# mankeyboy/ASR-FeatExt-OpenCL

Hardware: NVIDIA B200
Metric: mfcc_delta_delta2_frames_per_s (higher is better)
Workload: dtype f32

## Files before the change

asr-featext-opencl_b200/csrc/afe_batch.cu:

```cuda
#include <algorithm>
#include <atomic>
#include <memory>
#include <cmath>
#include <cstdlib>
#include <cstring>

#include "afe_internal.h"
#include "afe_fused_host.h"
#include "afe_nccl.h"

namespace afe {

void FftTables::build(int n2)
{
    release();
    N2 = n2;
    const int M = n2 / 2, R = M / 16;
    std::vector<float2> a((size_t)R * 16), p((size_t)M / 2);
    for (int l = 0; l < R; l++)
        for (int k1 = 0; k1 < 16; k1++) {
            const double ang = -2.0 * M_PI * (double)(l * k1) / (double)M;
            a[(size_t)l * 16 + k1] = make_float2((float)cos(ang), (float)sin(ang));
        }
    for (int k = 0; k < M / 2; k++) {
// ... 97 lines not shown

__global__ void k_normalize_tiles(float *__restrict__ out, const Tile *__restrict__ tiles, int width, int norm_type,
                                  const float *__restrict__ mean, const float *__restrict__ scale)
{
    extern __shared__ float s_ms[];
    dev::normalise_tile_rows(out, tiles[blockIdx.x], width, norm_type, mean, scale, s_ms);
}

static std::atomic<int> g_launches{0};
int kernel_launch_count() { return g_launches.load(); }
void count_launch(int n) { g_launches.fetch_add(n); }

#define AFE_DECL_INST(k) cudaError_t fused_launch_##k(const FusedLaunch &); int fused_max_clusters_##k(const FusedLaunch &);
#define AFE_FOR_EACH_INST(X) X(0) X(1) X(2) X(3) X(4) X(5) X(6) X(7) X(8) X(9) X(10) X(11) X(12) X(13) X(14) X(15) X(16) X(17) \
    X(18) X(19) X(20) X(21) X(22) X(23)
AFE_FOR_EACH_INST(AFE_DECL_INST)
#undef AFE_DECL_INST

cudaError_t launch_fused_variant(int key, const FusedLaunch &fl)
{
    typedef cudaError_t (*fn_t)(const FusedLaunch &);
#define AFE_ENTRY(k) fused_launch_##k,
    static const fn_t table[kFusedVariants] = {AFE_FOR_EACH_INST(AFE_ENTRY)};
#undef AFE_ENTRY
    if (key < 0 || key >= kFusedVariants) return cudaErrorInvalidValue;
    return table[key](fl);
}
int fused_variant_max_clusters(int key, const FusedLaunch &fl)
{
    typedef int (*fn_t)(const FusedLaunch &);
#define AFE_ENTRY(k) fused_max_clusters_##k,
    static const fn_t table[kFusedVariants] = {AFE_FOR_EACH_INST(AFE_ENTRY)};
#undef AFE_ENTRY
    if (key < 0 || key >= kFusedVariants) return -1;
    return table[key](fl);
}

std::string fused_unsupported_reason(const Derived &d)
{
    if (d.N2 != 512 && d.N2 != 256) return "fused path supports 256/512-point FFTs (window_size 129..512)";
    if (d.S % 2) return "fused path needs an even shift";
    if (d.dct_len > 16) return "fused path supports ceps_len + c0 <= 16";
    if (d.width > 128) return "fused path supports output width <= 128";
    if (d.nb > kMaxBanks) return "fused path supports num_banks <= 64";
    if (d.W > 26 * (d.M / 16) && d.W > d.N2) return "window longer than the FFT";
    return "";
}

static void build_mel_const(const Derived &d, float alpha, MelConst &mc)
{
    std::vector<int> edges; std::vector<float> filters, dct;
    build_filters(d, alpha, edges, filters);
    for (int i = 0; i + 1 < (int)edges.size(); i++)
        if (edges[i + 1] < edges[i]) throw Error("mel filter edges are not monotonic");
    if (edges.front() < 0 || edges.back() > d.M) throw Error("mel filterbank exceeds the Nyquist bin (check low_freq/high_freq)");
    memset(&mc, 0, sizeof mc);
    int off4 = 0;
    const float scale = 0.5f / (float)d.N2;
    for (int w = 0; w < 8; w++) {
        mc.wstart[w] = (short)off4;
        for (int b = w; b < d.nb; b += 8) {
            const int j0 = edges[b], j1 = edges[b + 2], s4 = j0 & ~3, n8 = std::max(1, (j1 - s4 + 7) / 8);
            if (off4 + 2 * n8 > kMaxWl4) throw Error("mel weight list exceeds the kernel-parameter budget");
            if (s4 + 8 * n8 > kMagStride + 16) throw Error("mel filter too wide for the fused kernel");
            mc.desc[b] = (s4 / 4) | (n8 << 16);
            float *wt = reinterpret_cast<float *>(mc.wl4 + off4);
            for (int j = j0; j < j1; j++) wt[j - s4] = filters[(size_t)(b % 2) * d.N2 + j] * scale;
            off4 += 2 * n8;
        }
    }
    if (d.C > 0) {
        build_dct(d, dct);
        for (int k = 0; k < d.nb; k++)
            for (int j = 0; j < d.dct_len; j++) reinterpret_cast<float *>(mc.dct4[k])[j] = dct[(size_t)k * d.dct_len + j];
    }
}

FusedEngine::FusedEngine(const Derived &dd, int dev) : d(dd), device(dev)
{
    const std::string why = fused_unsupported_reason(d);
    if (!why.empty()) throw Error(why);
    sm_count = sm_count_of(dev);
    fft.build(d.N2);
    int tc = 512;
    tc = std::min(tc, (6912 / d.cols) / kRoundFrames * kRoundFrames);
    tc = std::max(tc, kRoundFrames * ((2 * d.D + 1 + kRoundFrames - 1) / kRoundFrames + 1));
    tc_max = tc; nout_max = tc - 2 * d.D;
    const int ns = d.width / d.cols;
    L = d.N2 == 512 ? fused_smem_layout<512>(8, d.S, d.cols, tc_max, nout_max, d.l2, ns)
                    : fused_smem_layout<256>(8, d.S, d.cols, tc_max, nout_max, d.l2, ns);
    if (L.total > 227 * 1024) throw Error("fused kernel shared-memory budget exceeded");
    const int R = d.M / 16;
    pruned = d.W <= 26 * R;
    const int kf = (d.nb + 7) / 8;
    key = (d.N2 == 512 ? 0 : 6) + (pruned ? 0 : 3) + (kf <= 3 ? 0 : kf <= 5 ? 1 : 2);
}
FusedEngine::~FusedEngine() { fft.release(); mel.release(); }

void FusedEngine::set_window(const float *window, cudaStream_t st)
{
    upload_window(d, window, mel, st);
    window_set = true;
}
void FusedEngine::ensure_mel(float alpha)
{
    if (mc_alpha != alpha) { build_mel_const(d, alpha, mc); mc_alpha = alpha; }
}
std::string FusedEngine::kernel_label() const
{
    const int kf = (d.nb + 7) / 8;
    char buf[96];
    snprintf(buf, sizeof buf, "k_fused_mfcc<%d,%d,8,%d,%s>", d.N2, pruned ? 13 : 16, kf <= 3 ? 3 : kf <= 5 ? 5 : 8,
             pre != 0.f ? "true" : "false");
    return buf;
}

int FusedEngine::latency_tile(int n_out) const
{
    const int target = std::max(1, 2 * sm_count);
    const int want = (n_out + target - 1) / target;
    const int rounds = std::max(2, (want + 2 * d.D + kRoundFrames - 1) / kRoundFrames);
    return std::max(1, std::min(nout_max, rounds * kRoundFrames - 2 * d.D));
}

void FusedEngine::plan_uniform(int T, int t_first, int n_out, int nout_cap, int &ntile, int &nout) const
{
    const int cap = nout_cap > 0 ? std::min(nout_cap, nout_max) : nout_max;
    int best_cost = 1 << 30;
    ntile = (n_out + cap - 1) / cap;
    for (int cand = ntile; cand <= ntile + 3; cand++) {
        const int no = (n_out + cand - 1) / cand;
        int cost = 0;
        for (int t0 = t_first; t0 < t_first + n_out; t0 += no) {
            const int c0 = std::max(0, t0 - d.D), c1 = std::min(T, t0 + std::min(no, t_first + n_out - t0) + d.D);
            cost += (c1 - c0 + kRoundFrames - 1) / kRoundFrames;
        }
        if (cost < best_cost) { best_cost = cost; ntile = cand; }
    }
    nout = (n_out + ntile - 1) / ntile;
    ntile = (n_out + nout - 1) / nout;
}

int FusedEngine::plan_rows(std::vector<Tile> &tiles, long long pcm_off, long long out_row0, int T, int t_first, int n_out,
                           int group, int nout_cap) const
{
    if (n_out <= 0) return 0;
    int count, nout;
    plan_uniform(T, t_first, n_out, nout_cap, count, nout);
    const int first = (int)tiles.size();
    for (int t0 = t_first; t0 < t_first + n_out; t0 += nout) {
        Tile tl;
        tl.pcm_off = pcm_off; tl.out_row0 = out_row0; tl.T = T; tl.t0 = t0;
        tl.nout = std::min(nout, t_first + n_out - t0); tl.group = group;
        tl.tile0 = first; tl.ntiles = count; tl.flags = 0; tl.pad_ = 0;
        tiles.push_back(tl);
    }
    return count;
}

FusedArgs FusedEngine::base_args(int q1, bool use_tma) const
{
    FusedArgs a{};
    a.window2 = mel.d_window2; a.tw_a = fft.d_tw_a; a.tw_p = fft.d_tw_p;
    a.norm_type = d.p.norm; a.norm_after_dyn = d.p.norm_after_dyn;
    a.W = d.W; a.S = d.S; a.nb = d.nb; a.dct_len = d.C > 0 ? d.dct_len : 0; a.cols = d.cols; a.width = d.width;
    a.l1 = d.l1; a.l2 = d.l2; a.nstreams = d.width / d.cols;
    a.q1 = d.D > 0 ? q1 : 0;
    a.use_tma = use_tma ? 1 : 0;
    a.tc_max = tc_max;
    a.pre = pre;
    float den1 = 0, den2 = 0;
    for (int l = 1; l <= d.l1; l++) den1 += l * l;
    for (int l = 1; l <= d.l2; l++) den2 += l * l;
    a.rden1 = den1 > 0 ? 1.f / (2 * den1) : 0.f;
// ... 516 lines not shown
```

asr-featext-opencl_b200/csrc/afe_fused.cuh:

```cuda
#pragma once
#include <cfloat>

#include "afe_fft.cuh"
#include "afe_internal.h"
#include "afe_mel.cuh"

namespace afe {

struct Tile {
    long long pcm_off;
    long long out_row0;
    int T;
    int t0;
    int nout;
    int group;
    int tile0;
    int ntiles;
    int flags;
    int pad_;
};
constexpr int kTileNoStats = 1;
constexpr int kTileQ1All = 2;

constexpr int kMaxBanks = 64;
constexpr int kMaxWl4 = (2 * 257 + 10 * kMaxBanks + 3) / 4;
constexpr int kMagStride = 260;
__host__ __device__ constexpr int mag_row(int f) { return 8 * (f >> 3) + ((f >> 1) & 3) + 4 * (f & 1); }

struct MelConst {
    float4 wl4[kMaxWl4];
    float4 dct4[kMaxBanks][4];
    int desc[kMaxBanks];
    short wstart[8];
};

struct FusedArgs {
    const int16_t *pcm;
    float *out;
    const Tile *tiles;
    const float2 *window2, *tw_a, *tw_p;
    double *partials;
    int *counters;
    int cluster_norm;
    int tile_base;
    int norm_type, norm_after_dyn;
#ifdef AFE_DEVTOOLS
    int debug_skip;
#endif
    int W, S, nb, dct_len, cols, width, l1, l2, nstreams;
    int q1;
    int use_tma;
    int stats_rows_mode;
    int stats_count;
    int use_last;
    float *g_mean, *g_scale;
    int *work_counter;
    unsigned *flags;
    unsigned epoch;
    int ntiles_launch;
    float pre;
    int blk_ntiles, blk_T, blk_t_first, blk_n_out, blk_nout, blk_spec, blk_spec_q1;
    int stats_kind;
    int tc_max;
    float rden1, rden2;
};

constexpr int kRoundFrames = 32;
constexpr int kMaxFusedThreads = 256;

struct FusedSmem {
    int off_mbar, off_mags, off_part, off_warp, warp_bytes, w_pcm, w_scratch, pcm_bytes, off_dhat, off_dd, off_red,
        off_cep, total;
};

inline int align_up(int v, int a) { return (v + a - 1) / a * a; }

template <int N2>
FusedSmem fused_smem_layout(int kFusedWarps, int S, int cols, int tc_max, int nout_max, int l2, int nstreams)
{
    using C = dev::FftCfg<N2>;
    const int kWarpFrames = kRoundFrames / kFusedWarps;
    FusedSmem L;
    int o = 0;
    L.off_mbar = o; o += align_up(kFusedWarps * 8, 16);
    L.off_mags = o; o += align_up((kRoundFrames * kMagStride + 16) * 4, 16);
    L.pcm_bytes = align_up(((kWarpFrames - 1) * S + N2) * 2, 16) + 16;
    L.w_pcm = 0;
    L.warp_bytes = L.pcm_bytes;
    o = align_up(o, 128);
    L.off_warp = o; o += kFusedWarps * L.warp_bytes;
    o = align_up(o, 128);
    const int scratch = kFusedWarps * align_up(C::FPW * C::SCR * 8, 16);
    const int part = kFusedWarps * 4 * kRoundFrames * 16;
    L.w_scratch = align_up(C::FPW * C::SCR * 8, 16);
    L.off_part = o; o += scratch > part ? scratch : part;
    const int dhat = nstreams >= 2 ? align_up((nout_max + 2 * l2) * cols * 4, 16) : 0;
    const int dd = nstreams >= 3 ? align_up(nout_max * cols * 4, 16) : 0;
    L.off_dhat = L.off_mags;
    L.off_dd = L.off_dhat + dhat;
    L.off_red = L.off_dd + dd;
    const int phase3_end = L.off_red + kMaxFusedThreads * 4 * 8;
    if (phase3_end > o) o = align_up(phase3_end, 128);
    L.off_cep = o; o += align_up(tc_max * cols * 4, 16);
    L.total = o;
    return L;
}

namespace dev {

__device__ __forceinline__ uint32_t smem_u32(const void *p) { return (uint32_t)__cvta_generic_to_shared(p); }

__device__ __forceinline__ void mbar_init(uint64_t *bar, int count)
{
    asm volatile("mbarrier.init.shared::cta.b64 [%0], %1;" ::"r"(smem_u32(bar)), "r"(count));
}
__device__ __forceinline__ void mbar_expect_tx(uint64_t *bar, uint32_t bytes)
{
    asm volatile("mbarrier.arrive.expect_tx.shared::cta.b64 _, [%0], %1;" ::"r"(smem_u32(bar)), "r"(bytes) : "memory");
}
__device__ __forceinline__ void mbar_wait(uint64_t *bar, uint32_t parity)
{
    for (uint32_t spin = 0; spin < (1u << 24); spin++) {
        uint32_t done;
        asm volatile(
            "{\n\t.reg .pred p;\n\t"
            "mbarrier.try_wait.parity.shared::cta.b64 p, [%1], %2;\n\t"
            "selp.u32 %0, 1, 0, p;\n\t}"
            : "=r"(done)
            : "r"(smem_u32(bar)), "r"(parity)
            : "memory");
        if (done) return;
    }
    __trap();
}
__device__ __forceinline__ void tma_bulk_g2s(void *dst, const void *src, uint32_t bytes, uint64_t *bar)
{
    asm volatile("cp.async.bulk.shared::cluster.global.mbarrier::complete_tx::bytes [%0], [%1], %2, [%3];" ::"r"(
                     smem_u32(dst)),
                 "l"(src), "r"(bytes), "r"(smem_u32(bar))
                 : "memory");
}

__device__ __forceinline__ float4 lds128(uint32_t addr)
{
    float4 v;
    asm volatile("ld.shared.v4.f32 {%0, %1, %2, %3}, [%4];" : "=f"(v.x), "=f"(v.y), "=f"(v.z), "=f"(v.w) : "r"(addr));
    return v;
}
__device__ __forceinline__ uint32_t opaque(uint32_t v)
{
    asm volatile("" : "+r"(v));
    return v;
}

__device__ __forceinline__ void cluster_sync()
{
    asm volatile("barrier.cluster.arrive.release.aligned;\n\tbarrier.cluster.wait.acquire.aligned;" ::: "memory");
}
__device__ __forceinline__ uint32_t cluster_size()
{
    uint32_t n;
    asm volatile("mov.u32 %0, %%cluster_nctarank;" : "=r"(n));
    return n;
}
__device__ __forceinline__ double ld_peer_f64(const double *local, uint32_t rank)
{
    uint32_t peer;
    double v;
    asm volatile("mapa.shared::cluster.u32 %0, %1, %2;" : "=r"(peer) : "r"(smem_u32(local)), "r"(rank));
    asm volatile("ld.shared::cluster.f64 %0, [%1];" : "=d"(v) : "r"(peer) : "memory");
    return v;
}

__device__ __forceinline__ int clampi(int v, int lo, int hi) { return v < lo ? lo : (v > hi ? hi : v); }

template <class Dst>
__device__ __forceinline__ void sum_row_groups(const double *rec, int rp, int width, int c, Dst dst)
{
    double s0 = 0.0, s1 = 0.0, lo = (double)FLT_MAX, hi = -(double)FLT_MAX;
    for (int g = 0; g < rp; g++) {
        const double *p = rec + (g * width + c) * 4;
        s0 += p[0]; s1 += p[1];
        lo = fmin(lo, p[2]); hi = fmax(hi, p[3]);
    }
    double *d = dst();
    d[0] = s0; d[1] = s1; d[2] = lo; d[3] = hi;
}

}

namespace dev {

__device__ __forceinline__ float delta_num(const float *p, int stride, int L)
{
    if (L == 3) {
        float num = p[stride] - p[-stride];
        num = fmaf(2.f, p[2 * stride] - p[-2 * stride], num);
        return fmaf(3.f, p[3 * stride] - p[-3 * stride], num);
    }
    float num = 0.f;
    for (int l = 1; l <= L; l++) num = fmaf((float)l, p[l * stride] - p[-l * stride], num);
    return num;
}

template <int KIND>
__device__ __forceinline__ void write_rows(float *__restrict__ orow, const float *__restrict__ src, int r_off, int rpp, int nout,
                                           int rq, int rs, int cols, int width, int D, double &sum, double &sumsq, float &mn,
                                           float &mx)
{
    const int ostep = rpp * width, sstep = rpp * cols;
    orow += r_off * width;
    src += r_off * cols;
    for (int r = r_off; r < nout; r += rpp, orow += ostep, src += sstep) {
        const float sval = *src;
        *orow = r >= rq ? src[-D * cols] : sval;
        if (KIND >= 1 && r < rs) {
            sum += (double)sval;
            if (KIND >= 2) sumsq += (double)__fmul_rn(sval, sval);
            if (KIND >= 3) { mn = fminf(mn, sval); mx = fmaxf(mx, sval); }
        }
    }
}

template <int MODE>
__device__ __forceinline__ void phase3_l3(const int KIND, const FusedArgs &a, const Tile &tl, const float *__restrict__ s_cep,
                                          int c0f, int c1f, double *__restrict__ s_red3, int tid, int nthreads, int rs,
                                          const float *norm3 = nullptr)
{
    constexpr int R = 8;
    const int cols = a.cols, width = a.width, T = tl.T, t0 = tl.t0, nout = tl.nout;
    const int rp = nthreads / cols, g = tid / cols, c = tid - g * cols;
    if (g >= rp) return;
    const int q1 = (tl.flags & kTileQ1All) ? 2 : a.q1;
    const int rq = q1 ? (q1 == 2 ? 0 : max(0, T - 6 - t0)) : nout;
    const float rden1 = a.rden1, rden2 = a.rden2;
    double sum[3] = {0.0, 0.0, 0.0}, sumsq[3] = {0.0, 0.0, 0.0};
    float mn[3] = {FLT_MAX, FLT_MAX, FLT_MAX}, mx[3] = {-FLT_MAX, -FLT_MAX, -FLT_MAX};
    float nm[3] = {0.f, 0.f, 0.f}, ns[3] = {1.f, 1.f, 1.f};
    if (MODE == 2) {
#pragma unroll
        for (int k = 0; k < 3; k++) { nm[k] = norm3[k]; ns[k] = norm3[3 + k]; }
    }
    const bool cmn = a.norm_type == AFE_NORM_CMN;
    float *obase = a.out + (tl.out_row0 + t0) * (long long)width + c;
    for (int r0 = g * R; r0 < (MODE == 1 ? rs : nout); r0 += rp * R) {
        float x[R + 12], dh[R + 6];
#pragma unroll
        for (int i = 0; i < R + 12; i++)
            x[i] = s_cep[(clampi(t0 + r0 - 6 + i, c0f, c1f - 1) - c0f) * cols + c];
#pragma unroll
        for (int j = 0; j < R + 6; j++) {
            float num = x[j + 4] - x[j + 2];
            num = fmaf(2.f, x[j + 5] - x[j + 1], num);
            num = fmaf(3.f, x[j + 6] - x[j], num);
            dh[j] = __fmul_rn(num, rden1);
        }
        float *orow = obase + (long long)r0 * width;
#pragma unroll
        for (int r = 0; r < R; r++, orow += width) {
            const int row = r0 + r;
            if (row >= nout) break;
            float num = dh[r + 4] - dh[r + 2];
            num = fmaf(2.f, dh[r + 5] - dh[r + 1], num);
            num = fmaf(3.f, dh[r + 6] - dh[r], num);
            const float v[3] = {x[r + 6], dh[r + 3], __fmul_rn(num, rden2)};
            if (MODE == 0) {
                orow[0] = row >= rq ? x[r] : v[0];
                orow[cols] = v[1];
                orow[2 * cols] = v[2];
            } else if (MODE == 2) {
                const float w0 = row >= rq ? x[r] : v[0];
                orow[0] = cmn ? w0 - nm[0] : (w0 - nm[0]) * ns[0];
                orow[cols] = cmn ? v[1] - nm[1] : (v[1] - nm[1]) * ns[1];
                orow[2 * cols] = cmn ? v[2] - nm[2] : (v[2] - nm[2]) * ns[2];
            }
            if (MODE != 2 && KIND >= 1 && row < rs) {
#pragma unroll
                for (int k = 0; k < 3; k++) {
                    sum[k] += (double)v[k];
                    if (KIND >= 2) sumsq[k] += (double)__fmul_rn(v[k], v[k]);
                    if (KIND >= 3) { mn[k] = fminf(mn[k], v[k]); mx[k] = fmaxf(mx[k], v[k]); }
                }
            }
        }
    }
    if (MODE != 2) {
#pragma unroll
        for (int k = 0; k < 3; k++) {
            double *p = s_red3 + ((g * width) + k * cols + c) * 4;
            p[0] = sum[k]; p[1] = sumsq[k]; p[2] = (double)mn[k]; p[3] = (double)mx[k];
        }
    }
}

}

namespace dev {
__device__ __forceinline__ Tile load_tile(const FusedArgs &a, int idx)
{
    if (a.blk_ntiles == 0) return a.tiles[idx];
    const int D = a.l1 + a.l2;
    Tile tl;
    tl.pcm_off = 0; tl.out_row0 = -(long long)a.blk_t_first; tl.T = a.blk_T; tl.group = 0; tl.tile0 = 0;
    tl.ntiles = a.blk_ntiles + a.blk_spec; tl.pad_ = 0;
    if (idx < a.blk_ntiles) {
        tl.t0 = a.blk_t_first + idx * a.blk_nout;
        tl.nout = min(a.blk_nout, a.blk_t_first + a.blk_n_out - tl.t0);
        tl.flags = 0;
    } else {
        tl.t0 = a.blk_T - D; tl.nout = D;
        tl.flags = kTileNoStats | (a.blk_spec_q1 ? kTileQ1All : 0);
    }
    return tl;
}

constexpr int kSeqTiles = 32, kSegs = 6;
__host__ __device__ inline int seg_len(int ntiles) { return ntiles <= kSeqTiles ? ntiles : (ntiles + kSegs - 1) / kSegs; }

static __device__ unsigned g_opaque_zero = 0;

__device__ __forceinline__ void sum_records(const double *__restrict__ partials, int width, int c, int t_begin, int t_end,
                                            double &s0, double &s1, double &lo, double &hi, int tstep = 1)
{
    s0 = 0.0; s1 = 0.0; lo = (double)FLT_MAX; hi = -(double)FLT_MAX;
    constexpr int U = 8;
    const size_t stride = (size_t)width * 4 * tstep;
    const double *p = partials + ((size_t)t_begin * width + c) * 4;
    const int last = t_end - 1;
    const unsigned z = *reinterpret_cast<volatile unsigned *>(&g_opaque_zero);
    for (int t = t_begin; t < t_end; t += U * tstep, p += U * stride) {
        double2 a[U], b[U];
#pragma unroll
        for (int k = 0; k < U; k++) {
            const double2 *q = reinterpret_cast<const double2 *>(t + k * tstep <= last ? p + k * stride : p);
            a[k] = q[0];
            b[k] = q[1];
        }
        unsigned all = 0;
#pragma unroll
        for (int k = 0; k < U; k++)
            all |= (unsigned)__double2hiint(a[k].x) | (unsigned)__double2hiint(a[k].y) | (unsigned)__double2hiint(b[k].x) |
                   (unsigned)__double2hiint(b[k].y);
        a[0].x = __hiloint2double(__double2hiint(a[0].x) | (int)(all & z), __double2loint(a[0].x));
#pragma unroll
        for (int k = 0; k < U; k++) {
            const bool ok = t + k * tstep <= last;
            s0 += ok ? a[k].x : 0.0; s1 += ok ? a[k].y : 0.0;
            lo = fmin(lo, ok ? b[k].x : (double)FLT_MAX); hi = fmax(hi, ok ? b[k].y : -(double)FLT_MAX);
        }
    }
}

__device__ __forceinline__ void group_total(const double *__restrict__ partials, int width, int tile0, int ntiles, int tid,
                                            int nthreads, double *s_seg, int c_of_tid, double &s0, double &s1, double &lo, double &hi)
{
    if (ntiles <= kSeqTiles) {
        if (tid < width) sum_records(partials, width, c_of_tid, tile0, tile0 + ntiles, s0, s1, lo, hi);
        return;
    }
    const int len = seg_len(ntiles);
    for (int i = tid; i < kSegs * width; i += nthreads) {
        const int seg = i / width, c = i - seg * width;
        const int b = min(ntiles, seg * len), e = min(ntiles, b + len);
        double a0, a1, l, h;
        sum_records(partials, width, c, tile0 + b, tile0 + e, a0, a1, l, h);
        double *o = s_seg + (size_t)i * 4;
        o[0] = a0; o[1] = a1; o[2] = l; o[3] = h;
    }
    __syncthreads();
    if (tid < width) {
        s0 = 0.0; s1 = 0.0; lo = (double)FLT_MAX; hi = -(double)FLT_MAX;
        for (int seg = 0; seg < kSegs; seg++) {
            const double *o = s_seg + ((size_t)seg * width + c_of_tid) * 4;
            s0 += o[0]; s1 += o[1];
            lo = fmin(lo, o[2]); hi = fmax(hi, o[3]);
        }
    }
}

__device__ __forceinline__ void normalise_tile_rows(float *__restrict__ out, const Tile &tl, int width, int norm_type,
                                                    const float *__restrict__ mean, const float *__restrict__ scale, float *s_ms)
{
    float *base = out + (tl.out_row0 + tl.t0) * (long long)width;
    const int n = tl.nout * width;
    for (int i = threadIdx.x; i < width; i += blockDim.x) {
        s_ms[i] = __ldcg(mean + (long long)tl.group * width + i);
        s_ms[width + i] = norm_type == AFE_NORM_CMN ? 1.f : __ldcg(scale + (long long)tl.group * width + i);
    }
    __syncthreads();
    const float *m = s_ms, *sc = s_ms + width;
    const bool cmn = norm_type == AFE_NORM_CMN;
    const int head = min(n, (int)(((16 - (reinterpret_cast<uintptr_t>(base) & 15)) & 15) >> 2));
    const int n4 = (n - head) >> 2, tail0 = head + 4 * n4;
    if ((int)threadIdx.x < head) {
        const int i = threadIdx.x;
        const float v = __ldcg(base + i) - m[i % width];
        base[i] = cmn ? v : v * sc[i % width];
    }
    if ((int)threadIdx.x < n - tail0) {
        const int i = tail0 + threadIdx.x, c = i % width;
        const float v = __ldcg(base + i) - m[c];
        base[i] = cmn ? v : v * sc[c];
    }
    float4 *p4 = reinterpret_cast<float4 *>(base + head);
    int c = (head + 4 * (int)threadIdx.x) % width;
    const int cstep = (4 * (int)blockDim.x) % width;
    constexpr int U = 4;
    const int bd = blockDim.x;
    for (int j = threadIdx.x; j < n4; j += U * bd) {
        float4 v[U];
#pragma unroll
        for (int k = 0; k < U; k++)
            if (j + k * bd < n4) v[k] = __ldcg(p4 + j + k * bd);
#pragma unroll
        for (int k = 0; k < U; k++) {
            if (j + k * bd < n4) {
                int c1 = c + 1; if (c1 >= width) c1 -= width;
                int c2 = c1 + 1; if (c2 >= width) c2 -= width;
                int c3 = c2 + 1; if (c3 >= width) c3 -= width;
                float4 w = v[k];
                w.x -= m[c]; w.y -= m[c1]; w.z -= m[c2]; w.w -= m[c3];
                if (!cmn) { w.x *= sc[c]; w.y *= sc[c1]; w.z *= sc[c2]; w.w *= sc[c3]; }
                p4[j + k * bd] = w;
            }
            c += cstep; if (c >= width) c -= width;
        }
    }
}

__device__ __forceinline__ void normalise_role(const FusedArgs &a, const Tile tl, float *s_ms)
{
    if (threadIdx.x == 0) {
        unsigned v = 0;
        for (unsigned spin = 0; spin < (1u << 26); spin++) {
            asm volatile("ld.acquire.gpu.global.u32 %0, [%1];" : "=r"(v) : "l"(a.flags + tl.group) : "memory");
            if (v == a.epoch) break;
            __nanosleep(128);
        }
        if (v != a.epoch) __trap();
    }
    __syncthreads();
    normalise_tile_rows(a.out, tl, a.width, a.norm_type, a.g_mean, a.g_scale, s_ms);
}
}

template <int N2, int NZ, int kFusedWarps, int KF, bool PRE>
__global__ void __launch_bounds__(32 * kFusedWarps, 2)
k_fused_mfcc(const FusedArgs a, const FusedSmem L, const __grid_constant__ MelConst mc)
{
    constexpr bool FAST = false;
    using C = dev::FftCfg<N2>;
    constexpr int kFusedThreads = 32 * kFusedWarps, kWarpFrames = kRoundFrames / kFusedWarps;
    constexpr int R = C::R, FPW = C::FPW, SCR = C::SCR;
    static_assert(kWarpFrames % FPW == 0, "a warp's frames must fill whole FFT calls");
    extern __shared__ __align__(128) unsigned char smem[];
    float *s_mags = reinterpret_cast<float *>(smem + L.off_mags);
    float *s_cep = reinterpret_cast<float *>(smem + L.off_cep);

    const int tid = threadIdx.x, lane = tid & 31;
    const int warp = __shfl_sync(0xffffffffu, tid >> 5, 0);
    const int lf = lane % R, fw = lane / R;
    unsigned char *wbase = smem + L.off_warp + warp * L.warp_bytes;
    uint64_t *w_mbar = reinterpret_cast<uint64_t *>(smem + L.off_mbar) + warp;
    unsigned char *w_pcm = wbase + L.w_pcm;
    float2 *w_scratch = reinterpret_cast<float2 *>(smem + L.off_part + warp * L.w_scratch);

    int tile_local = blockIdx.x;
    if (a.work_counter) {
        __shared__ int s_role;
        if (tid == 0) {
            const int t = atomicAdd(a.work_counter, 1);
            if (t == (int)gridDim.x - 1) *a.work_counter = 0;
            s_role = t;
        }
        __syncthreads();
        tile_local = s_role;
        if (tile_local >= a.ntiles_launch) {
            const int n_norm = (int)gridDim.x - a.ntiles_launch;
            for (int j = tile_local - a.ntiles_launch; j < a.ntiles_launch; j += n_norm) {
                dev::normalise_role(a, dev::load_tile(a, a.tile_base + j), reinterpret_cast<float *>(smem));
                __syncthreads();
            }
            return;
        }
    }
    const int tile_idx = a.tile_base + tile_local;
    const Tile tl = dev::load_tile(a, tile_idx);
    const int q1 = (tl.flags & kTileQ1All) ? 2 : a.q1;
    const int D = a.l1 + a.l2, cols = a.cols;
    const int c0f = max(0, tl.t0 - D), c1f = min(tl.T, tl.t0 + tl.nout + D);
    const int ncomp = c1f - c0f;
    const int nrounds = (ncomp + kRoundFrames - 1) / kRoundFrames;
    const int16_t *wpcm = a.pcm + tl.pcm_off + (long long)(c0f + warp * kWarpFrames) * a.S;
    auto warp_frames = [&](int r) { return min(kWarpFrames, ncomp - r * kRoundFrames - warp * kWarpFrames); };
    auto issue_tma = [&](int r) {
        const int nf = warp_frames(r);
        if (nf <= 0) return;
        const uint32_t bytes = (uint32_t)((((nf - 1) * a.S + a.W) * 2 + 15) & ~15);
        asm volatile("fence.proxy.async.shared::cta;" ::: "memory");
        dev::mbar_expect_tx(w_mbar, bytes);
        dev::tma_bulk_g2s(w_pcm, wpcm + (long long)r * kRoundFrames * a.S, bytes, w_mbar);
    };
    if (a.use_tma && lane == 0) {
        dev::mbar_init(w_mbar, 1);
        asm volatile("fence.mbarrier_init.release.cluster;" ::: "memory");
        issue_tma(0);
    }
    dev::LaneConsts<N2, NZ> lc;
    dev::load_lane_consts<N2, NZ>(lc, a.window2, a.tw_a, a.tw_p, lf);
    for (int i = tid; i < (kRoundFrames * kMagStride + 16) / 4; i += kFusedThreads)
// ... 67 lines not shown
                        acc0 = __ffma2_rn(make_float2(m0.x, m0.y), make_float2(w0.x, w0.y), acc0);
                        acc1 = __ffma2_rn(make_float2(m0.z, m0.w), make_float2(w0.z, w0.w), acc1);
                        acc0 = __ffma2_rn(make_float2(m1.x, m1.y), make_float2(w1.x, w1.y), acc0);
                        acc1 = __ffma2_rn(make_float2(m1.z, m1.w), make_float2(w1.z, w1.w), acc1);
                        woff += 2;
                        if (--n8 == 0) break;
                        maddr += 32;
                        m0 = dev::lds128(maddr);
                        m1 = dev::lds128(maddr + 16);
                    }
                }
                const float2 t = __fadd2_rn(acc0, acc1);
                es[k] = t.x + t.y;
            }
#pragma unroll
            for (int k = 0; k + 1 < KF; k += 2) {
                const float2 e2 = dev::mel_log2<FAST>(make_float2(es[k], es[k + 1]));
                es[k] = e2.x; es[k + 1] = e2.y;
            }
            if (KF & 1) es[KF - 1] = dev::mel_log<FAST>(es[KF - 1]);
            if (a.dct_len > 0) {
                float2 cep[8];
#pragma unroll
                for (int c = 0; c < 8; c++) cep[c] = make_float2(0.f, 0.f);
#pragma unroll
                for (int k = 0; k < KF; k++) {
                    const int b = warp + k * kFusedWarps;
                    const float2 e2 = make_float2(es[k], es[k]);
#pragma unroll
                    for (int c4 = 0; c4 < 4; c4++) {
                        const float4 d4 = mc.dct4[b][c4];
                        cep[2 * c4 + 0] = __ffma2_rn(e2, make_float2(d4.x, d4.y), cep[2 * c4 + 0]);
                        cep[2 * c4 + 1] = __ffma2_rn(e2, make_float2(d4.z, d4.w), cep[2 * c4 + 1]);
                    }
                }
#pragma unroll
                for (int c4 = 0; c4 < 4; c4++)
                    reinterpret_cast<float4 *>(smem + L.off_part + c4 * L.w_scratch)[warp * kRoundFrames + lane] =
                        make_float4(cep[2 * c4].x, cep[2 * c4].y, cep[2 * c4 + 1].x, cep[2 * c4 + 1].y);
            } else {
#pragma unroll
                for (int k = 0; k < KF; k++)
                    if (warp + k * kFusedWarps < a.nb) s_cep[(f0 + lane) * cols + warp + k * kFusedWarps] = es[k];
            }
        }
        __syncthreads();
        if (a.dct_len > 0 && warp < 4) {
            if (lane < nfr) {
                const float4 *part = reinterpret_cast<const float4 *>(w_scratch);
                float4 t = part[lane];
#pragma unroll
                for (int w2 = 1; w2 < kFusedWarps; w2++) {
                    const float4 u = part[w2 * kRoundFrames + lane];
                    t.x += u.x; t.y += u.y; t.z += u.z; t.w += u.w;
                }
                float *crow = s_cep + (f0 + lane) * cols + 4 * warp;
                if (4 * warp + 0 < a.dct_len) crow[0] = t.x;
                if (4 * warp + 1 < a.dct_len) crow[1] = t.y;
                if (4 * warp + 2 < a.dct_len) crow[2] = t.z;
                if (4 * warp + 3 < a.dct_len) crow[3] = t.w;
            }
            __syncwarp();
        }
    }
    __syncthreads();

    float *s_dhat = reinterpret_cast<float *>(smem + L.off_dhat);
    float *s_dd = reinterpret_cast<float *>(smem + L.off_dd);
    double *s_red = reinterpret_cast<double *>(smem + L.off_red);
    const int T = tl.T, t0 = tl.t0, nout = tl.nout, l1 = a.l1, l2 = a.l2;
#ifdef AFE_DEVTOOLS
    if (a.debug_skip & 4) return;
#endif
    const int width = a.width;
    const int rpp = kFusedThreads / width;
    const bool active = tid < rpp * width;
    const int r_off = tid / width, col = tid - r_off * width;
    const int strm = col / cols, c = col - strm * cols;
    const int n_stats = a.stats_rows_mode == 1 ? T - D : a.stats_rows_mode == 2 ? T : a.stats_rows_mode == 3 ? a.stats_count : 0;
    const float *src = strm == 0 ? s_cep + (t0 - c0f) * cols + c : strm == 1 ? s_dhat + l2 * cols + c : s_dd + c;
    const int rq = (q1 && strm == 0) ? (q1 == 2 ? 0 : max(0, T - D - t0)) : nout;
    const int rs = (tl.flags & kTileNoStats) ? 0 : a.stats_rows_mode == 3 ? nout : min(nout, max(0, n_stats - t0));
    const bool fast3 = a.nstreams == 3 && l1 == 3 && l2 == 3;
    if (fast3 && a.use_last) {
        const int cc = tid % cols;
        const float *gm = a.g_mean + (long long)tl.group * width, *gs = a.g_scale + (long long)tl.group * width;
        const float norm3[6] = {gm[cc], gm[cols + cc], gm[2 * cols + cc], gs[cc], gs[cols + cc], gs[2 * cols + cc]};
        dev::phase3_l3<2>(0, a, tl, s_cep, c0f, c1f, nullptr, tid, kFusedThreads, rs, norm3);
    } else if (fast3 && a.cluster_norm) {
        double *s_red3 = reinterpret_cast<double *>(smem + L.off_mags);
        double *s_rec = reinterpret_cast<double *>(smem + L.off_mags + 25 * 1024);
        float *s_mean = reinterpret_cast<float *>(smem + L.off_mags + 30 * 1024), *s_scale = s_mean + width;
        dev::phase3_l3<1>(a.stats_kind, a, tl, s_cep, c0f, c1f, s_red3, tid, kFusedThreads, rs);
        __syncthreads();
        if (tid < width) dev::sum_row_groups(s_red3, kFusedThreads / cols, width, tid, [&] { return s_rec + tid * 4; });
        dev::cluster_sync();
        if (tid < width) {
            const double *rec = s_rec + (a.norm_after_dyn ? tid : tid % cols) * 4;
            const uint32_t ncta = dev::cluster_size();
            double s0 = 0.0, s1 = 0.0, lo = (double)FLT_MAX, hi = -(double)FLT_MAX;
            for (uint32_t t = 0; t < ncta; t++) {
                s0 += dev::ld_peer_f64(rec, t); s1 += dev::ld_peer_f64(rec + 1, t);
                lo = fmin(lo, dev::ld_peer_f64(rec + 2, t)); hi = fmax(hi, dev::ld_peer_f64(rec + 3, t));
            }
            float m, sc;
            finalize_column(a.norm_type, (double)n_stats, s0, s1, (float)lo, (float)hi, m, sc);
            if (!a.norm_after_dyn && tid >= cols) m = 0.f;
            s_mean[tid] = m; s_scale[tid] = sc;
            if (a.g_mean && tile_idx == tl.tile0) {
                a.g_mean[(long long)tl.group * width + tid] = m;
                a.g_scale[(long long)tl.group * width + tid] = sc;
            }
        }
        __syncthreads();
        {
            const int cc = tid % cols;
            const float norm3[6] = {s_mean[cc], s_mean[cols + cc], s_mean[2 * cols + cc],
                                    s_scale[cc], s_scale[cols + cc], s_scale[2 * cols + cc]};
            dev::phase3_l3<2>(0, a, tl, s_cep, c0f, c1f, s_red3, tid, kFusedThreads, rs, norm3);
        }
        dev::cluster_sync();
    } else if (fast3) {
        double *s_red3 = reinterpret_cast<double *>(smem + L.off_mags);
        dev::phase3_l3<0>(a.stats_kind, a, tl, s_cep, c0f, c1f, s_red3, tid, kFusedThreads, rs);
        if (a.partials) {
            __syncthreads();
            if (tid < width)
                dev::sum_row_groups(s_red3, kFusedThreads / cols, width, tid, [&] { return a.partials + ((long long)tile_idx * width + tid) * 4; });
        }
    } else {
        if (a.nstreams >= 2) {
            const int rp = kFusedThreads / cols, rl = tid / cols, c = tid - rl * cols;
            const int nd = nout + 2 * l2;
            if (rl < rp) {
                for (int i = rl; i < nd; i += rp) {
                    const int u = t0 - l2 + i;
                    float num;
                    if (u - l1 >= 0 && u + l1 <= T - 1)
                        num = dev::delta_num(s_cep + (u - c0f) * cols + c, cols, l1);
                    else {
                        num = 0.f;
                        for (int l = 1; l <= l1; l++) {
                            const float hi = s_cep[(dev::clampi(u + l, 0, T - 1) - c0f) * cols + c];
                            const float lo = s_cep[(dev::clampi(u - l, 0, T - 1) - c0f) * cols + c];
                            num = fmaf((float)l, hi - lo, num);
                        }
                    }
                    s_dhat[i * cols + c] = num * a.rden1;
                }
            }
            __syncthreads();
            if (a.nstreams >= 3) {
                if (rl < rp)
                    for (int r = rl; r < nout; r += rp)
                        s_dd[r * cols + c] = dev::delta_num(s_dhat + (r + l2) * cols + c, cols, l2) * a.rden2;
                __syncthreads();
            }
        }

        double sum = 0.0, sumsq = 0.0;
        float mn = FLT_MAX, mx = -FLT_MAX;
        if (active) {
            float *orow = a.out + (tl.out_row0 + t0) * (long long)width + col;
            switch (a.stats_kind) {
            case 0: dev::write_rows<0>(orow, src, r_off, rpp, nout, rq, rs, cols, width, D, sum, sumsq, mn, mx); break;
            case 1: dev::write_rows<1>(orow, src, r_off, rpp, nout, rq, rs, cols, width, D, sum, sumsq, mn, mx); break;
            case 2: dev::write_rows<2>(orow, src, r_off, rpp, nout, rq, rs, cols, width, D, sum, sumsq, mn, mx); break;
            default: dev::write_rows<3>(orow, src, r_off, rpp, nout, rq, rs, cols, width, D, sum, sumsq, mn, mx); break;
            }
        }
        if (a.partials) {
            s_red[tid * 4 + 0] = sum;
            s_red[tid * 4 + 1] = sumsq;
            s_red[tid * 4 + 2] = (double)mn;
            s_red[tid * 4 + 3] = (double)mx;
            __syncthreads();
            if (tid < width)
                dev::sum_row_groups(s_red, rpp, width, tid, [&] { return a.partials + ((long long)tile_idx * width + tid) * 4; });
        }
        if (a.use_last) {
            __syncthreads();
            dev::normalise_tile_rows(a.out, tl, width, a.norm_type, a.g_mean, a.g_scale, reinterpret_cast<float *>(smem + L.off_dhat));
        }
    }

    if (a.counters) {
        __shared__ int s_last;
        float *s_mean = reinterpret_cast<float *>(smem + L.off_dhat), *s_scale = s_mean + width;
        __threadfence();
        __syncthreads();
        if (tid == 0) {
            const int ticket = atomicAdd(a.counters + tl.group, 1);
            s_last = ticket == tl.ntiles - 1;
            if (s_last) a.counters[tl.group] = 0;
        }
        __syncthreads();
        if (s_last) {
            __threadfence();
            double s0, s1, lo, hi;
            {
                double *s_seg = reinterpret_cast<double *>(smem + L.off_mags + 1024);
                const int src_col = a.norm_after_dyn ? tid : tid % cols;
                dev::group_total(a.partials, width, tl.tile0, tl.ntiles, tid, kFusedThreads, s_seg, tid < width ? src_col : 0, s0, s1, lo, hi);
            }
            if (tid < width) {
                float m, sc;
                finalize_column(a.norm_type, (double)n_stats, s0, s1, (float)lo, (float)hi, m, sc);
                if (!a.norm_after_dyn && tid >= cols) m = 0.f;
                s_mean[tid] = m; s_scale[tid] = sc;
                if (a.g_mean) {
                    a.g_mean[(long long)tl.group * width + tid] = m;
// ... 35 lines not shown
```

Measured before the change: 1.596 billion.

## Stage fused delta rows in shared memory and normalise with vectorised stores

The fused MFCC+delta+delta2 path now writes the computed rows of a tile into a shared-memory staging buffer, instead of writing them to global memory or recomputing them. The normalised output is then emitted with aligned float4 stores. In the cluster-normalisation mode this replaces a second full recomputation pass of the delta/delta2 stencil with a copy from shared memory. The final cluster barrier is split into arrive and wait so the store overlaps the peers' progress. It costs extra shared memory, chosen by a layout search, and adds a check that occupancy of 2 CTAs per SM is not lost.

```diff
diff --git a/asr-featext-opencl_b200/csrc/afe_batch.cu b/asr-featext-opencl_b200/csrc/afe_batch.cu
--- a/asr-featext-opencl_b200/csrc/afe_batch.cu
+++ b/asr-featext-opencl_b200/csrc/afe_batch.cu
@@ -203,14 +203,16 @@
     if (!why.empty()) throw Error(why);
     sm_count = sm_count_of(dev);
     fft.build(d.N2);
-    int tc = 512;
-    tc = std::min(tc, (6912 / d.cols) / kRoundFrames * kRoundFrames);
-    tc = std::max(tc, kRoundFrames * ((2 * d.D + 1 + kRoundFrames - 1) / kRoundFrames + 1));
-    tc_max = tc; nout_max = tc - 2 * d.D;
+    fused_tile_capacity(d.cols, d.D, tc_max, nout_max);
     const int ns = d.width / d.cols;
-    L = d.N2 == 512 ? fused_smem_layout<512>(8, d.S, d.cols, tc_max, nout_max, d.l2, ns)
-                    : fused_smem_layout<256>(8, d.S, d.cols, tc_max, nout_max, d.l2, ns);
+    const bool staged = ns == 3 && d.l1 == 3 && d.l2 == 3;
+    L = d.N2 == 512 ? fused_smem_layout<512>(8, d.S, d.cols, tc_max, nout_max, d.l2, ns, staged)
+                    : fused_smem_layout<256>(8, d.S, d.cols, tc_max, nout_max, d.l2, ns, staged);
     if (L.total > 227 * 1024) throw Error("fused kernel shared-memory budget exceeded");
+    const FusedSmem Lg = d.N2 == 512 ? fused_smem_layout<512>(8, d.S, d.cols, tc_max, nout_max, d.l2, ns, false)
+                                     : fused_smem_layout<256>(8, d.S, d.cols, tc_max, nout_max, d.l2, ns, false);
+    if (L.total > kFusedSmem2Cta && Lg.total <= kFusedSmem2Cta)
+        throw Error("internal error: the fused kernel's staged rows do not fit 2 CTAs per SM");
     const int R = d.M / 16;
     pruned = d.W <= 26 * R;
     const int kf = (d.nb + 7) / 8;
diff --git a/asr-featext-opencl_b200/csrc/afe_fused.cuh b/asr-featext-opencl_b200/csrc/afe_fused.cuh
--- a/asr-featext-opencl_b200/csrc/afe_fused.cuh
+++ b/asr-featext-opencl_b200/csrc/afe_fused.cuh
@@ -1,4 +1,5 @@
 #pragma once
+#include <algorithm>
 #include <cfloat>
 
 #include "afe_fft.cuh"
@@ -70,13 +71,24 @@
 
 struct FusedSmem {
     int off_mbar, off_mags, off_part, off_warp, warp_bytes, w_pcm, w_scratch, pcm_bytes, off_dhat, off_dd, off_red,
-        off_cep, total;
+        off_cep, off_stage, off_red3, off_rec, total;
 };
 
 inline int align_up(int v, int a) { return (v + a - 1) / a * a; }
 
+constexpr int kFusedSmem2Cta = 228 * 1024 / 2 - 1024 - 128;
+
+inline void fused_tile_capacity(int cols, int D, int &tc_max, int &nout_max)
+{
+    int tc = 512;
+    tc = tc < (6912 / cols) / kRoundFrames * kRoundFrames ? tc : (6912 / cols) / kRoundFrames * kRoundFrames;
+    const int lo = kRoundFrames * ((2 * D + 1 + kRoundFrames - 1) / kRoundFrames + 1);
+    tc_max = tc > lo ? tc : lo;
+    nout_max = tc_max - 2 * D;
+}
+
 template <int N2>
-FusedSmem fused_smem_layout(int kFusedWarps, int S, int cols, int tc_max, int nout_max, int l2, int nstreams)
+FusedSmem fused_smem_layout(int kFusedWarps, int S, int cols, int tc_max, int nout_max, int l2, int nstreams, bool staged)
 {
     using C = dev::FftCfg<N2>;
     const int kWarpFrames = kRoundFrames / kFusedWarps;
@@ -101,8 +113,23 @@
     L.off_red = L.off_dd + dd;
     const int phase3_end = L.off_red + kMaxFusedThreads * 4 * 8;
     if (phase3_end > o) o = align_up(phase3_end, 128);
-    L.off_cep = o; o += align_up(tc_max * cols * 4, 16);
-    L.total = o;
+    const int width = cols * nstreams;
+    const int stage = staged ? align_up(nout_max * width * 4 + 16, 16) : 0;
+    const int red3 = staged ? (kFusedWarps * 32 / cols) * width * 32 : 0, rec = staged ? width * 40 : 0;
+    const int cep = align_up(tc_max * cols * 4, 16);
+    L.off_stage = L.off_mags;
+    const int stage_end = L.off_stage + stage, dead_end = o;
+    int best = 0, best_total = 0;
+    for (int k = 0; k < 3; k++) {
+        const int behind = (k == 0 ? red3 : 0) + (k != 1 ? rec : 0), over = red3 + rec - behind;
+        const int t = std::max(dead_end, align_up(stage_end + behind, 128)) + std::max(cep, over);
+        if (k == 0 || t < best_total) { best = k; best_total = t; }
+    }
+    o = std::max(dead_end, align_up(stage_end + (best == 0 ? red3 : 0) + (best != 1 ? rec : 0), 128));
+    L.off_cep = o;
+    L.off_red3 = best == 0 ? stage_end : L.off_cep;
+    L.off_rec = best == 0 ? stage_end + red3 : best == 1 ? L.off_cep + red3 : stage_end;
+    L.total = best_total;
     return L;
 }
 
@@ -157,6 +184,8 @@
 {
     asm volatile("barrier.cluster.arrive.release.aligned;\n\tbarrier.cluster.wait.acquire.aligned;" ::: "memory");
 }
+__device__ __forceinline__ void cluster_arrive() { asm volatile("barrier.cluster.arrive.release.aligned;" ::: "memory"); }
+__device__ __forceinline__ void cluster_wait() { asm volatile("barrier.cluster.wait.acquire.aligned;" ::: "memory"); }
 __device__ __forceinline__ uint32_t cluster_size()
 {
     uint32_t n;
@@ -222,28 +251,20 @@
     }
 }
 
-template <int MODE>
 __device__ __forceinline__ void phase3_l3(const int KIND, const FusedArgs &a, const Tile &tl, const float *__restrict__ s_cep,
-                                          int c0f, int c1f, double *__restrict__ s_red3, int tid, int nthreads, int rs,
-                                          const float *norm3 = nullptr)
+                                          int c0f, int c1f, float *__restrict__ rows, double *__restrict__ s_red3, int tid,
+                                          int nthreads, int rs)
 {
     constexpr int R = 8;
     const int cols = a.cols, width = a.width, T = tl.T, t0 = tl.t0, nout = tl.nout;
     const int rp = nthreads / cols, g = tid / cols, c = tid - g * cols;
-    if (g >= rp) return;
     const int q1 = (tl.flags & kTileQ1All) ? 2 : a.q1;
     const int rq = q1 ? (q1 == 2 ? 0 : max(0, T - 6 - t0)) : nout;
     const float rden1 = a.rden1, rden2 = a.rden2;
     double sum[3] = {0.0, 0.0, 0.0}, sumsq[3] = {0.0, 0.0, 0.0};
     float mn[3] = {FLT_MAX, FLT_MAX, FLT_MAX}, mx[3] = {-FLT_MAX, -FLT_MAX, -FLT_MAX};
-    float nm[3] = {0.f, 0.f, 0.f}, ns[3] = {1.f, 1.f, 1.f};
-    if (MODE == 2) {
-#pragma unroll
-        for (int k = 0; k < 3; k++) { nm[k] = norm3[k]; ns[k] = norm3[3 + k]; }
-    }
-    const bool cmn = a.norm_type == AFE_NORM_CMN;
-    float *obase = a.out + (tl.out_row0 + t0) * (long long)width + c;
-    for (int r0 = g * R; r0 < (MODE == 1 ? rs : nout); r0 += rp * R) {
+    float *sbase = rows + c;
+    for (int r0 = g * R; g < rp && r0 < nout; r0 += rp * R) {
         float x[R + 12], dh[R + 6];
 #pragma unroll
         for (int i = 0; i < R + 12; i++)
@@ -255,26 +276,19 @@
             num = fmaf(3.f, x[j + 6] - x[j], num);
             dh[j] = __fmul_rn(num, rden1);
         }
-        float *orow = obase + (long long)r0 * width;
-#pragma unroll
-        for (int r = 0; r < R; r++, orow += width) {
+        float *srow = sbase + r0 * width;
+#pragma unroll
+        for (int r = 0; r < R; r++, srow += width) {
             const int row = r0 + r;
             if (row >= nout) break;
             float num = dh[r + 4] - dh[r + 2];
             num = fmaf(2.f, dh[r + 5] - dh[r + 1], num);
             num = fmaf(3.f, dh[r + 6] - dh[r], num);
             const float v[3] = {x[r + 6], dh[r + 3], __fmul_rn(num, rden2)};
-            if (MODE == 0) {
-                orow[0] = row >= rq ? x[r] : v[0];
-                orow[cols] = v[1];
-                orow[2 * cols] = v[2];
-            } else if (MODE == 2) {
-                const float w0 = row >= rq ? x[r] : v[0];
-                orow[0] = cmn ? w0 - nm[0] : (w0 - nm[0]) * ns[0];
-                orow[cols] = cmn ? v[1] - nm[1] : (v[1] - nm[1]) * ns[1];
-                orow[2 * cols] = cmn ? v[2] - nm[2] : (v[2] - nm[2]) * ns[2];
-            }
-            if (MODE != 2 && KIND >= 1 && row < rs) {
+            srow[0] = row >= rq ? x[r] : v[0];
+            srow[cols] = v[1];
+            srow[2 * cols] = v[2];
+            if (KIND >= 1 && row < rs) {
 #pragma unroll
                 for (int k = 0; k < 3; k++) {
                     sum[k] += (double)v[k];
@@ -284,7 +298,8 @@
             }
         }
     }
-    if (MODE != 2) {
+    __syncthreads();
+    if (g < rp) {
 #pragma unroll
         for (int k = 0; k < 3; k++) {
             double *p = s_red3 + ((g * width) + k * cols + c) * 4;
@@ -378,54 +393,69 @@
     }
 }
 
-__device__ __forceinline__ void normalise_tile_rows(float *__restrict__ out, const Tile &tl, int width, int norm_type,
-                                                    const float *__restrict__ mean, const float *__restrict__ scale, float *s_ms)
-{
-    float *base = out + (tl.out_row0 + tl.t0) * (long long)width;
-    const int n = tl.nout * width;
+template <bool STAGED>
+__device__ __forceinline__ void store_tile_rows(float *dst, const float *src, int n, int width, const float *m,
+                                                const float *sc, bool cmn)
+{
+    auto ld = [&](int i) { return STAGED ? src[i] : __ldcg(src + i); };
+    auto ld4 = [&](int j) {
+        const float4 *s4 = reinterpret_cast<const float4 *>(src);
+        return STAGED ? s4[j] : __ldcg(s4 + j);
+    };
+    auto apply = [&](float v, int c) { return cmn ? v - m[c] : (v - m[c]) * sc[c]; };
+    const int tid = threadIdx.x;
+    const int head = min(n, (int)(((16 - (reinterpret_cast<uintptr_t>(dst) & 15)) & 15) >> 2));
+    const int n4 = (n - head) >> 2, tail0 = head + 4 * n4;
+    if (tid < head) dst[tid] = apply(ld(tid), tid % width);
+    if (tid < n - tail0) {
+        const int i = tail0 + tid;
+        dst[i] = apply(ld(i), i % width);
+    }
+    src += head;
+    float4 *p4 = reinterpret_cast<float4 *>(dst + head);
+    const int period = width / ((width & 3) == 0 ? 4 : (width & 1) == 0 ? 2 : 1);
+    const int nt = (int)blockDim.x / period * period;
+    if (tid >= nt) return;
+    const int c0 = (head + 4 * tid) % width;
+    int c1 = c0 + 1; if (c1 >= width) c1 -= width;
+    int c2 = c1 + 1; if (c2 >= width) c2 -= width;
+    int c3 = c2 + 1; if (c3 >= width) c3 -= width;
+    const float4 mv = make_float4(m[c0], m[c1], m[c2], m[c3]);
+    const float4 sv = cmn ? make_float4(1.f, 1.f, 1.f, 1.f) : make_float4(sc[c0], sc[c1], sc[c2], sc[c3]);
+    constexpr int U = 4;
+    for (int j = tid; j < n4; j += U * nt) {
+        float4 v[U];
+#pragma unroll
+        for (int k = 0; k < U; k++)
+            if (j + k * nt < n4) v[k] = ld4(j + k * nt);
+#pragma unroll
+        for (int k = 0; k < U; k++) {
+            if (j + k * nt < n4) {
+                float4 w = v[k];
+                w.x -= mv.x; w.y -= mv.y; w.z -= mv.z; w.w -= mv.w;
+                if (!cmn) { w.x *= sv.x; w.y *= sv.y; w.z *= sv.z; w.w *= sv.w; }
+                p4[j + k * nt] = w;
+            }
+        }
+    }
+}
+
+__device__ __forceinline__ void load_group_norm(const Tile &tl, int width, int norm_type, const float *__restrict__ mean,
+                                                const float *__restrict__ scale, float *s_ms)
+{
     for (int i = threadIdx.x; i < width; i += blockDim.x) {
         s_ms[i] = __ldcg(mean + (long long)tl.group * width + i);
         s_ms[width + i] = norm_type == AFE_NORM_CMN ? 1.f : __ldcg(scale + (long long)tl.group * width + i);
     }
+}
+
+__device__ __forceinline__ void normalise_tile_rows(float *__restrict__ out, const Tile &tl, int width, int norm_type,
+                                                    const float *__restrict__ mean, const float *__restrict__ scale, float *s_ms)
+{
+    float *base = out + (tl.out_row0 + tl.t0) * (long long)width;
+    load_group_norm(tl, width, norm_type, mean, scale, s_ms);
     __syncthreads();
-    const float *m = s_ms, *sc = s_ms + width;
-    const bool cmn = norm_type == AFE_NORM_CMN;
-    const int head = min(n, (int)(((16 - (reinterpret_cast<uintptr_t>(base) & 15)) & 15) >> 2));
-    const int n4 = (n - head) >> 2, tail0 = head + 4 * n4;
-    if ((int)threadIdx.x < head) {
-        const int i = threadIdx.x;
-        const float v = __ldcg(base + i) - m[i % width];
-        base[i] = cmn ? v : v * sc[i % width];
-    }
-    if ((int)threadIdx.x < n - tail0) {
-        const int i = tail0 + threadIdx.x, c = i % width;
-        const float v = __ldcg(base + i) - m[c];
-        base[i] = cmn ? v : v * sc[c];
-    }
-    float4 *p4 = reinterpret_cast<float4 *>(base + head);
-    int c = (head + 4 * (int)threadIdx.x) % width;
-    const int cstep = (4 * (int)blockDim.x) % width;
-    constexpr int U = 4;
-    const int bd = blockDim.x;
-    for (int j = threadIdx.x; j < n4; j += U * bd) {
-        float4 v[U];
-#pragma unroll
-        for (int k = 0; k < U; k++)
-            if (j + k * bd < n4) v[k] = __ldcg(p4 + j + k * bd);
-#pragma unroll
-        for (int k = 0; k < U; k++) {
-            if (j + k * bd < n4) {
-                int c1 = c + 1; if (c1 >= width) c1 -= width;
-                int c2 = c1 + 1; if (c2 >= width) c2 -= width;
-                int c3 = c2 + 1; if (c3 >= width) c3 -= width;
-                float4 w = v[k];
-                w.x -= m[c]; w.y -= m[c1]; w.z -= m[c2]; w.w -= m[c3];
-                if (!cmn) { w.x *= sc[c]; w.y *= sc[c1]; w.z *= sc[c2]; w.w *= sc[c3]; }
-                p4[j + k * bd] = w;
-            }
-            c += cstep; if (c >= width) c -= width;
-        }
-    }
+    store_tile_rows<false>(base, base, tl.nout * width, width, s_ms, s_ms + width, norm_type == AFE_NORM_CMN);
 }
 
 __device__ __forceinline__ void normalise_role(const FusedArgs &a, const Tile tl, float *s_ms)
@@ -659,51 +689,51 @@
     const int rq = (q1 && strm == 0) ? (q1 == 2 ? 0 : max(0, T - D - t0)) : nout;
     const int rs = (tl.flags & kTileNoStats) ? 0 : a.stats_rows_mode == 3 ? nout : min(nout, max(0, n_stats - t0));
     const bool fast3 = a.nstreams == 3 && l1 == 3 && l2 == 3;
-    if (fast3 && a.use_last) {
-        const int cc = tid % cols;
-        const float *gm = a.g_mean + (long long)tl.group * width, *gs = a.g_scale + (long long)tl.group * width;
-        const float norm3[6] = {gm[cc], gm[cols + cc], gm[2 * cols + cc], gs[cc], gs[cols + cc], gs[2 * cols + cc]};
-        dev::phase3_l3<2>(0, a, tl, s_cep, c0f, c1f, nullptr, tid, kFusedThreads, rs, norm3);
-    } else if (fast3 && a.cluster_norm) {
-        double *s_red3 = reinterpret_cast<double *>(smem + L.off_mags);
-        double *s_rec = reinterpret_cast<double *>(smem + L.off_mags + 25 * 1024);
-        float *s_mean = reinterpret_cast<float *>(smem + L.off_mags + 30 * 1024), *s_scale = s_mean + width;
-        dev::phase3_l3<1>(a.stats_kind, a, tl, s_cep, c0f, c1f, s_red3, tid, kFusedThreads, rs);
-        __syncthreads();
-        if (tid < width) dev::sum_row_groups(s_red3, kFusedThreads / cols, width, tid, [&] { return s_rec + tid * 4; });
-        dev::cluster_sync();
-        if (tid < width) {
-            const double *rec = s_rec + (a.norm_after_dyn ? tid : tid % cols) * 4;
-            const uint32_t ncta = dev::cluster_size();
-            double s0 = 0.0, s1 = 0.0, lo = (double)FLT_MAX, hi = -(double)FLT_MAX;
-            for (uint32_t t = 0; t < ncta; t++) {
-                s0 += dev::ld_peer_f64(rec, t); s1 += dev::ld_peer_f64(rec + 1, t);
-                lo = fmin(lo, dev::ld_peer_f64(rec + 2, t)); hi = fmax(hi, dev::ld_peer_f64(rec + 3, t));
-            }
-            float m, sc;
-            finalize_column(a.norm_type, (double)n_stats, s0, s1, (float)lo, (float)hi, m, sc);
-            if (!a.norm_after_dyn && tid >= cols) m = 0.f;
-            s_mean[tid] = m; s_scale[tid] = sc;
-            if (a.g_mean && tile_idx == tl.tile0) {
-                a.g_mean[(long long)tl.group * width + tid] = m;
-                a.g_scale[(long long)tl.group * width + tid] = sc;
-            }
-        }
-        __syncthreads();
-        {
-            const int cc = tid % cols;
-            const float norm3[6] = {s_mean[cc], s_mean[cols + cc], s_mean[2 * cols + cc],
-                                    s_scale[cc], s_scale[cols + cc], s_scale[2 * cols + cc]};
-            dev::phase3_l3<2>(0, a, tl, s_cep, c0f, c1f, s_red3, tid, kFusedThreads, rs, norm3);
-        }
-        dev::cluster_sync();
-    } else if (fast3) {
-        double *s_red3 = reinterpret_cast<double *>(smem + L.off_mags);
-        dev::phase3_l3<0>(a.stats_kind, a, tl, s_cep, c0f, c1f, s_red3, tid, kFusedThreads, rs);
-        if (a.partials) {
+    if (fast3) {
+        float *o_tile = a.out + (tl.out_row0 + t0) * (long long)width;
+        float *stage = reinterpret_cast<float *>(smem + L.off_stage) + ((reinterpret_cast<uintptr_t>(o_tile) >> 2) & 3);
+        const int rp3 = kFusedThreads / cols;
+        double *s_red3 = reinterpret_cast<double *>(smem + L.off_red3);
+        double *s_rec = reinterpret_cast<double *>(smem + L.off_rec);
+        float *s_mean = reinterpret_cast<float *>(s_rec + width * 4), *s_scale = s_mean + width;
+        const bool cmn = a.norm_type == AFE_NORM_CMN;
+        if (a.use_last || a.cluster_norm)
+            dev::phase3_l3(a.stats_kind, a, tl, s_cep, c0f, c1f, stage, s_red3, tid, kFusedThreads, rs);
+        else
+            dev::phase3_l3(a.stats_kind, a, tl, s_cep, c0f, c1f, o_tile, s_red3, tid, kFusedThreads, rs);
+        if (a.use_last) {
+            dev::load_group_norm(tl, width, a.norm_type, a.g_mean, a.g_scale, s_mean);
+            __syncthreads();
+            dev::store_tile_rows<true>(o_tile, stage, nout * width, width, s_mean, s_scale, cmn);
+        } else if (a.cluster_norm) {
+            __syncthreads();
+            if (tid < width) dev::sum_row_groups(s_red3, rp3, width, tid, [&] { return s_rec + tid * 4; });
+            dev::cluster_sync();
+            if (tid < width) {
+                const double *rec = s_rec + (a.norm_after_dyn ? tid : tid % cols) * 4;
+                const uint32_t ncta = dev::cluster_size();
+                double s0 = 0.0, s1 = 0.0, lo = (double)FLT_MAX, hi = -(double)FLT_MAX;
+                for (uint32_t t = 0; t < ncta; t++) {
+                    s0 += dev::ld_peer_f64(rec, t); s1 += dev::ld_peer_f64(rec + 1, t);
+                    lo = fmin(lo, dev::ld_peer_f64(rec + 2, t)); hi = fmax(hi, dev::ld_peer_f64(rec + 3, t));
+                }
+                float m, sc;
+                finalize_column(a.norm_type, (double)n_stats, s0, s1, (float)lo, (float)hi, m, sc);
+                if (!a.norm_after_dyn && tid >= cols) m = 0.f;
+                s_mean[tid] = m; s_scale[tid] = sc;
+                if (a.g_mean && tile_idx == tl.tile0) {
+                    a.g_mean[(long long)tl.group * width + tid] = m;
+                    a.g_scale[(long long)tl.group * width + tid] = sc;
+                }
+            }
+            dev::cluster_arrive();
+            __syncthreads();
+            dev::store_tile_rows<true>(o_tile, stage, nout * width, width, s_mean, s_scale, cmn);
+            dev::cluster_wait();
+        } else if (a.partials) {
             __syncthreads();
             if (tid < width)
-                dev::sum_row_groups(s_red3, kFusedThreads / cols, width, tid, [&] { return a.partials + ((long long)tile_idx * width + tid) * 4; });
+                dev::sum_row_groups(s_red3, rp3, width, tid, [&] { return a.partials + ((long long)tile_idx * width + tid) * 4; });
         }
     } else {
         if (a.nstreams >= 2) {
```

After: 1.633 billion, median of 6. +2.3%, better.
